# DoubangoTelecom/compv

Hardware: AMD Instinct MI355X
Metric: Mpixels/s Sobel->Canny->HoughSHT on 4K uint8 (higher is better)
Workload: dtype u8; 1 GPU; batched 3840x2160 uint8 frames, Sobel3x3 -> Canny(59,119) -> HoughSHT(rho=1, theta=1deg, thr=100); 256 distinct frames resident per GPU as 8 batches of 32, a step processes one batch, steps rotate over the batches; frames_per_gpu=32, resident_batches=8, parallelism=frames sharded across 1 GPU(s), no data-path collective

## Files before the change

compv_amd/csrc/api.cpp:

```cpp
#include "../../include/compv_hip.h"
#include "kernels.hpp"
#include "kht.hpp"

#include <atomic>
#include <chrono>
#include <condition_variable>
#include <deque>
#include <functional>
#include <mutex>
#include <thread>

#include <hip/hip_runtime.h>
#if defined(__linux__)
#include <sched.h>
#endif

#include <algorithm>
#include <cmath>
#include <cstdio>
#include <cstdlib>
#include <cstring>
#include <string>
#include <memory>
#include <vector>
// ... 101 lines not shown
};

struct StepParams {
	const uint8_t* d_in = nullptr; float tLow = 0.f, tHigh = 0.f; int threshold = 0, maxLines = 0;
	int ksize = 3, thresholdType = COMPVHIP_CANNY_THRESHOLD_COMPARE_TO_GRADIENT, pixfmt = COMPVHIP_FMT_Y;
	uint8_t* d_gray = nullptr; int32_t* d_otsu = nullptr; float* d_cart = nullptr;
	uint8_t* d_edges = nullptr; compvhip_line* d_lines = nullptr; size_t lineCap = 0; int32_t* d_counts = nullptr;
};

struct compvhip_plan : TimingState {
	compvhip_ctx* ctx = nullptr;
	size_t W = 0, H = 0, S = 0, frames = 0;
	float thetaDeg = 1.f;
	int tilesX = 0, tilesY = 0, wb = 0;
	size_t bitsFrameStride = 0;
	uint32_t* ebits = nullptr; uint32_t* ubits = nullptr;
	int* counters = nullptr;
	size_t nCounts = 0;
	int* flags = nullptr; int* hFlags = nullptr;
	int* frameTotals = nullptr; unsigned int* lineTotal = nullptr;
	unsigned int* hTotals = nullptr;
	unsigned int recentTotals[8] = {}; int recentN = 0;
	int specRounds = kSpecRounds; unsigned char recentRounds[8] = {}; int recentRoundsN = 0;
	int* hRoundsDev = nullptr; int* stepHostSlot = nullptr;
	int* hRounds = nullptr;
	int roundsUsed = 0;
	int maxRounds = kMaxRounds;
	bool countersFresh = false;
	int2* thrDev = nullptr; unsigned int* sums = nullptr;
	uint8_t* dirty = nullptr;
	uint8_t* patchOut = nullptr; uint8_t* copyBack = nullptr;
	uint8_t* grayTmp = nullptr;
	uint8_t* tmpOut = nullptr;
	bool bitsValid = false;
	bool shtReady = false;
	size_t R = 0, T = 0; float thetaStep = 0.f; int accPitch = 0;
	uint8_t* blurTmp = nullptr;
	uint32_t* hist = nullptr; int32_t* otsu = nullptr;
	float* cosT = nullptr; float* invSinT = nullptr;
	int32_t* sinQ = nullptr; int32_t* cosQ = nullptr;
	uint32_t* edges = nullptr; size_t edgeCap = 0; int* edgeCounts = nullptr;
	uint16_t* acc = nullptr; size_t accFrameStride = 0;
	uint32_t* keysA = nullptr; uint32_t* keysB = nullptr; uint32_t* valsA = nullptr; uint32_t* valsB = nullptr; size_t lineCap = 0; int* lineCounts = nullptr;
	int2* reach = nullptr;
	int2* nmsRange = nullptr;
	uint8_t* nmsFlags = nullptr;
	int* blockCounts = nullptr; int lineBlocks = 0;
	void* sortTemp = nullptr; size_t sortTempBytes = 0;
	int32_t* segPerLine = nullptr; size_t segPerLineCap = 0;
	int32_t* compRows = nullptr; uint32_t* compBits = nullptr; int32_t* compParent = nullptr;
	uint8_t* morphTmp = nullptr;
	int* fastWork = nullptr; uint8_t* fastScores = nullptr;
	int strengthBits = 16, keyBits = 0;
	uint16_t* chunkHist = nullptr; uint32_t* strengthStart = nullptr; int sortChunks = 0; bool deviceSort = false;
	bool voteTiles = false;
	ShtTileArgs vt = {};
	std::vector<int32_t> vtKt, vtRowBase;
	int32_t* dKt = nullptr; int32_t* dRowBase = nullptr; uint8_t* partLo = nullptr; uint8_t* partHi = nullptr; uint8_t* colFlag = nullptr; int* tileCounts = nullptr;
	std::vector<KhtBatchState*> khtBatch;
	std::vector<std::unique_ptr<KhtPeaksWork>> khtWork;
	double khtStageMs[6] = {}; double khtWallMs = 0.0; int khtThreads = 0;
	struct AsyncStep { bool used = false; bool replay = false; uint64_t seq = 0; hipEvent_t done = nullptr; hipStream_t stream = nullptr; StepParams sp; size_t sortN = 0; int rounds = 0; } steps[kAsyncDepth];
	uint64_t stepSeq = 0;
};

struct compvhip_matcher : TimingState {
	compvhip_ctx* ctx = nullptr;
	int descDwords = 0, queryCap = 0, trainCap = 0, pairs = 0, knn = 0;
	uint32_t* partial = nullptr;
	compvhip_match* reverse = nullptr;
};

namespace {

int fail(compvhip_ctx* ctx, int code, const char* what, hipError_t e = hipSuccess)
{
	if (ctx) {
		ctx->err = what ? what : "";
		if (e != hipSuccess) { ctx->err += ": "; ctx->err += hipGetErrorString(e); }
	}
	return code;
}

#define HIPCHK(ctx, call) do { hipError_t e__ = (call); if (e__ != hipSuccess) return fail((ctx), COMPVHIP_E_HIP, #call, e__); } while (0)

template <typename T>
hipError_t dmalloc(compvhip_ctx* ctx, T** p, size_t count)
{
	*p = nullptr;
	if (!count) return hipSuccess;
	hipError_t e = hipMalloc(reinterpret_cast<void**>(p), count * sizeof(T));
	if (e == hipSuccess && ctx) ctx->live++;
	return e;
}
template <typename T>
void dfree(compvhip_ctx* ctx, T*& p)
{
	if (p) { (void)hipFree(p); if (ctx) ctx->live--; p = nullptr; }
}

size_t alignUp(size_t v, size_t a) { return (v + a - 1) / a * a; }

void khtScratchFree(compvhip_ctx* ctx, KhtScratch& k)
{
	dfree(ctx, k.counts); dfree(ctx, k.params); dfree(ctx, k.cells); dfree(ctx, k.cellCount);
	dfree(ctx, k.pts); dfree(ctx, k.spans); dfree(ctx, k.kernelsDev);
	dfree(ctx, k.strings); dfree(ctx, k.counts32); dfree(ctx, k.scratch); dfree(ctx, k.stack);
// ... 263 lines not shown
				for (int i = 0; i < tiles; ++i) {
					const int b = p->vtRowBase[static_cast<size_t>(i) * T + t];
					lo = std::min(lo, b); hi = std::max(hi, b + Rw);
				}
				reach[t] = make_int2(lo, hi);
			}
			dfree(ctx, p->reach);
			HIPCHK(ctx, dmalloc(ctx, &p->reach, reach.size()));
			HIPCHK(ctx, hipMemcpy(p->reach, reach.data(), reach.size() * sizeof(int2), hipMemcpyHostToDevice));
			dfree(ctx, p->nmsRange);
			HIPCHK(ctx, dmalloc(ctx, &p->nmsRange, range.size()));
			HIPCHK(ctx, hipMemcpy(p->nmsRange, range.data(), range.size() * sizeof(int2), hipMemcpyHostToDevice));
		}
		HIPCHK(ctx, dmalloc(ctx, &p->dKt, p->vtKt.size()));
		HIPCHK(ctx, dmalloc(ctx, &p->dRowBase, p->vtRowBase.size()));
		HIPCHK(ctx, hipMemcpy(p->dKt, p->vtKt.data(), p->vtKt.size() * sizeof(int32_t), hipMemcpyHostToDevice));
		HIPCHK(ctx, hipMemcpy(p->dRowBase, p->vtRowBase.data(), p->vtRowBase.size() * sizeof(int32_t), hipMemcpyHostToDevice));
		{
			const size_t cols = p->frames * p->vt.tiles * static_cast<size_t>(p->vt.Tpad);
			HIPCHK(ctx, dmalloc(ctx, &p->partLo, cols * p->vt.rwPitch));
			HIPCHK(ctx, dmalloc(ctx, &p->partHi, cols * p->vt.rwPitch));
			HIPCHK(ctx, dmalloc(ctx, &p->colFlag, cols));
		}
		p->vt.kt = p->dKt; p->vt.rowBase = p->dRowBase; p->vt.partLo = p->partLo; p->vt.partHi = p->partHi; p->vt.colFlag = p->colFlag; p->vt.reach = p->reach; p->vt.tileCounts = p->tileCounts;
		p->edgeCap = static_cast<size_t>(p->vt.tiles) * p->vt.tileCap;
	}
	HIPCHK(ctx, dmalloc(ctx, &p->edges, p->edgeCap * p->frames));
	HIPCHK(ctx, dmalloc(ctx, &p->acc, p->accFrameStride * p->frames));
	HIPCHK(ctx, hipMemset(p->acc, 0, sizeof(uint16_t) * p->accFrameStride * p->frames));
	p->strengthBits = 1;
	while ((static_cast<size_t>(1) << p->strengthBits) <= 2 * (p->W > p->H ? p->W : p->H)) p->strengthBits++;
	if (p->strengthBits > 16) p->strengthBits = 16;
	int frameBits = 0;
	while ((static_cast<size_t>(1) << frameBits) < p->frames) frameBits++;
	p->keyBits = frameBits + p->strengthBits;
	if (R * T >= (static_cast<size_t>(1) << 32)) return fail(ctx, COMPVHIP_E_INVALID_PARAMETER, "theta step too small: the accumulator has 2^32 cells or more");
	if (p->keyBits > 32) return fail(ctx, COMPVHIP_E_INVALID_PARAMETER, "too many frames for a 32-bit line key");
	dfree(ctx, p->nmsFlags);
	{
		const size_t frows = sht_nms_rows(static_cast<int>(R)), fgroups = static_cast<size_t>(sht_nms_groups(static_cast<int>(T)));
		HIPCHK(ctx, dmalloc(ctx, &p->nmsFlags, frows * fgroups * p->frames));
		HIPCHK(ctx, hipMemset(p->nmsFlags, 0, frows * fgroups * p->frames));
		if (sht_lines_blocks(static_cast<int>(R)) != p->lineBlocks) return fail(ctx, COMPVHIP_E_INVALID_STATE, "row-block counters were sized for another accumulator");
	}
	p->shtReady = true;
	return COMPVHIP_OK;
}

int ensureLineCap(compvhip_plan* p, size_t cap)
{
	compvhip_ctx* ctx = p->ctx;
	cap = std::min(cap, p->R * p->T);
	if (cap <= p->lineCap) return COMPVHIP_OK;
	dfree(ctx, p->keysA); dfree(ctx, p->keysB); dfree(ctx, p->valsA); dfree(ctx, p->valsB); dfree(ctx, p->sortTemp); dfree(ctx, p->chunkHist); dfree(ctx, p->strengthStart);
	p->lineCap = 0; p->deviceSort = false;
	HIPCHK(ctx, dmalloc(ctx, &p->keysA, cap * p->frames));
	HIPCHK(ctx, dmalloc(ctx, &p->keysB, cap * p->frames));
	HIPCHK(ctx, dmalloc(ctx, &p->valsA, cap * p->frames));
	HIPCHK(ctx, dmalloc(ctx, &p->valsB, cap * p->frames));
	size_t tb = 0;
	hipError_t e = sht_sort_pairs(nullptr, tb, p->keysA, p->keysB, p->valsA, p->valsB, cap * p->frames, p->keyBits, nullptr);
	if (e != hipSuccess) return fail(ctx, COMPVHIP_E_HIP, "radix sort size query", e);
	p->sortTempBytes = tb;
	uint8_t* tmp = nullptr;
	HIPCHK(ctx, dmalloc(ctx, &tmp, std::max<size_t>(tb, 16)));
	p->sortTemp = tmp;
	p->sortChunks = static_cast<int>((cap + kShtSortChunk - 1) / kShtSortChunk);
	if (p->strengthBits <= kShtSortMaxStrengthBits && p->sortChunks <= kShtSortMaxChunks) {
		HIPCHK(ctx, dmalloc(ctx, &p->chunkHist, p->frames * static_cast<size_t>(p->sortChunks) << kShtSortMaxStrengthBits));
		HIPCHK(ctx, dmalloc(ctx, &p->strengthStart, p->frames << kShtSortMaxStrengthBits));
		p->deviceSort = true;
	}
	p->lineCap = cap;
	p->recentN = 0;
	return COMPVHIP_OK;
}

ShtArgs shtArgs(compvhip_plan* p, int threshold)
{
	ShtArgs a;
	a.ebits = p->ebits; a.edges = p->edges; a.edgeCounts = p->edgeCounts; a.acc = p->acc;
	a.sinQ = p->sinQ; a.cosQ = p->cosQ; a.lineKeys = p->keysA; a.lineVals = p->valsA; a.lineCounts = p->lineCounts;
	a.frameTotals = p->frameTotals; a.lineTotal = p->lineTotal; a.sortN = 0; a.outCounts = nullptr; a.stepFlags = nullptr; a.hostStep = nullptr;
	a.nmsRange = p->nmsRange; a.blockCounts = p->blockCounts; a.lineBlocks = p->lineBlocks; a.nmsFlags = p->nmsFlags; a.nmsRows = static_cast<int>(sht_nms_rows(static_cast<int>(p->R))); a.nmsGroups = sht_nms_groups(static_cast<int>(p->T));
	a.bitsFrameStride = p->bitsFrameStride; a.edgeCap = p->edgeCap; a.accFrameStride = p->accFrameStride; a.lineCap = p->lineCap;
	a.W = static_cast<int>(p->W); a.H = static_cast<int>(p->H); a.wb = p->wb;
	a.R = static_cast<int>(p->R); a.T = static_cast<int>(p->T); a.accPitch = p->accPitch; a.barrier = static_cast<int>(p->W + p->H);
	a.threshold = threshold;
	a.nmsLastCol = static_cast<int>((p->T - 1) & ~static_cast<size_t>(3));
	a.frames = static_cast<int>(p->frames);
	a.strengthBits = p->strengthBits;
	return a;
}

int ensurePreproc(compvhip_plan* p)
{
	compvhip_ctx* ctx = p->ctx;
	if (!p->hist) HIPCHK(ctx, dmalloc(ctx, &p->hist, static_cast<size_t>(256) * kOtsuMaxChunks * p->frames));
	if (!p->otsu) HIPCHK(ctx, dmalloc(ctx, &p->otsu, p->frames));
	return COMPVHIP_OK;
}

int enqueueCanny(compvhip_plan* p, const uint8_t* d_in, uint8_t* d_out, int tLow, int tHigh, int ksize, int thrMode, float fLow, float fHigh, hipStream_t st)
{
	compvhip_ctx* ctx = p->ctx;
	CannyArgs a;
	a.zero = nullptr; a.nZero = 0;
	a.in = d_in; a.out = d_out; a.ebits = p->ebits; a.ubits = p->ubits; a.thrDev = (thrMode != COMPVHIP_CANNY_THRESHOLD_COMPARE_TO_GRADIENT) ? p->thrDev : nullptr;
	a.inFrameStride = p->S * p->H; a.outFrameStride = p->S * p->H; a.bitsFrameStride = p->bitsFrameStride;
	a.W = static_cast<int>(p->W); a.H = static_cast<int>(p->H); a.S = static_cast<int>(p->S); a.So = static_cast<int>(p->S);
	a.wb = p->wb; a.tilesX = p->tilesX; a.tilesY = p->tilesY; a.tLow = tLow; a.tHigh = tHigh; a.ksize = ksize;
	cannyCoverage(p->W, &a.simdEnd, &a.cStart);
	const bool gap = !((a.simdEnd >= a.W - 1) || (a.cStart <= a.simdEnd));
	if (thrMode == COMPVHIP_CANNY_THRESHOLD_OTSU) {
		int rc = ensurePreproc(p);
		if (rc) return rc;
		Stamp s(p, st, "otsu_kernels");
		HIPCHK(ctx, launch_otsu(d_in, a.W, a.H, a.S, a.inFrameStride, static_cast<int>(p->frames), fLow, fHigh, p->hist, p->otsu, p->thrDev, st));
	}
	if (thrMode == COMPVHIP_CANNY_THRESHOLD_PERCENT_OF_MEAN) {
		Stamp s(p, st, "canny_mean_thresholds");
		HIPCHK(ctx, launch_mean_thresholds(d_in, a.W, a.H, a.S, a.inFrameStride, static_cast<int>(p->frames), fLow, fHigh, p->sums, p->thrDev, st));
	}
// ... 320 lines not shown
		if (hipMemset(p->ebits, 0, sizeof(uint32_t) * p->bitsFrameStride * frames) != hipSuccess) { rc = COMPVHIP_E_HIP; break; }
		if (hipMemset(p->ubits, 0, sizeof(uint32_t) * p->bitsFrameStride * frames) != hipSuccess) { rc = COMPVHIP_E_HIP; break; }
		if (hipDeviceSynchronize() != hipSuccess) { rc = COMPVHIP_E_HIP; break; }
		{
			p->voteTiles = true;
			size_t R = 0, T = 0; float step = 0.f;
			if (p->voteTiles && shtDims(W, H, thetaDeg, &R, &T, &step) == COMPVHIP_OK && T >= 5) {
				std::vector<int32_t> sq, cq;
				shtTables(thetaDeg, T, sq, cq);
				if (!planVoteTiles(W, H, frames, sq, cq, p->vt, p->vtKt, p->vtRowBase)) p->voteTiles = false;
			}
			else p->voteTiles = false;
			p->lineBlocks = p->voteTiles ? sht_lines_blocks(static_cast<int>(R)) : 0;
			p->nCounts = (2 + static_cast<size_t>(p->voteTiles ? p->vt.tiles : 0) + static_cast<size_t>(p->lineBlocks)) * frames + (frames + 1) * kFrameSlot;
		}
		if (dmalloc(ctx, &p->counters, p->nCounts + kMaxRounds) != hipSuccess) { rc = COMPVHIP_E_OUT_OF_MEMORY; break; }
		p->edgeCounts = p->counters; p->lineCounts = p->counters + frames; p->tileCounts = p->counters + 2 * frames; p->blockCounts = p->counters + (2 + static_cast<size_t>(p->voteTiles ? p->vt.tiles : 0)) * frames; p->flags = p->counters + p->nCounts;
		p->frameTotals = p->blockCounts + static_cast<size_t>(p->lineBlocks) * frames; p->lineTotal = reinterpret_cast<unsigned int*>(p->frameTotals + frames * kFrameSlot);
		if (const char* e = getenv("COMPVHIP_RESOLVE_WRAP")) { const int v = atoi(e); if (v >= 8 && v <= kMaxRounds && (v & 3) == 0) p->maxRounds = v; }
		if (hipMemset(p->counters, 0, sizeof(int) * (p->nCounts + kMaxRounds)) != hipSuccess) { rc = COMPVHIP_E_HIP; break; }
		if (dmalloc(ctx, &p->thrDev, frames) != hipSuccess) { rc = COMPVHIP_E_OUT_OF_MEMORY; break; }
		if (dmalloc(ctx, &p->dirty, canny_resolve_dirty_bytes(static_cast<int>(H), p->wb, static_cast<int>(frames))) != hipSuccess) { rc = COMPVHIP_E_OUT_OF_MEMORY; break; }
		if (dmalloc(ctx, &p->sums, frames * kFrameSlot) != hipSuccess) { rc = COMPVHIP_E_OUT_OF_MEMORY; break; }
		if (hipHostMalloc(reinterpret_cast<void**>(&p->hFlags), sizeof(int) * 2 * (kAsyncDepth + 1)) != hipSuccess) { rc = COMPVHIP_E_OUT_OF_MEMORY; break; }
		p->hTotals = reinterpret_cast<unsigned int*>(p->hFlags + kAsyncDepth + 1);
		if (hipHostMalloc(reinterpret_cast<void**>(&p->hRounds), sizeof(int) * (kFrameSlot + 4) * kAsyncDepth, hipHostMallocMapped) != hipSuccess) { rc = COMPVHIP_E_OUT_OF_MEMORY; break; }
		if (hipHostGetDevicePointer(reinterpret_cast<void**>(&p->hRoundsDev), p->hRounds, 0) != hipSuccess) { rc = COMPVHIP_E_HIP; break; }
	} while (0);
	if (rc) { compvhip_plan_destroy(p); return fail(ctx, rc, "plan allocation"); }
	*out = p;
	return COMPVHIP_OK;
}

void compvhip_plan_destroy(compvhip_plan* p)
{
	if (!p) return;
	compvhip_ctx* ctx = p->ctx;
	(void)hipSetDevice(ctx->device);
	timelineClear(p);
	for (hipEvent_t e : p->eventPool) (void)hipEventDestroy(e);
	for (auto& stp : p->steps) if (stp.done) (void)hipEventDestroy(stp.done);
	dfree(ctx, p->dirty);
	dfree(ctx, p->ebits); dfree(ctx, p->ubits); dfree(ctx, p->counters); dfree(ctx, p->thrDev); dfree(ctx, p->sums); dfree(ctx, p->tmpOut);
	if (p->hFlags) (void)hipHostFree(p->hFlags);
	if (p->hRounds) (void)hipHostFree(p->hRounds);
	dfree(ctx, p->hist); dfree(ctx, p->otsu); dfree(ctx, p->blurTmp); dfree(ctx, p->grayTmp);
	dfree(ctx, p->morphTmp);
	dfree(ctx, p->fastWork); dfree(ctx, p->fastScores);
	for (KhtBatchState* b : p->khtBatch) khtBatchFree(ctx, b);
	p->khtBatch.clear();
	dfree(ctx, p->cosT); dfree(ctx, p->invSinT);
	dfree(ctx, p->dKt); dfree(ctx, p->dRowBase); dfree(ctx, p->partLo); dfree(ctx, p->partHi); dfree(ctx, p->colFlag);
	dfree(ctx, p->sinQ); dfree(ctx, p->cosQ); dfree(ctx, p->edges); dfree(ctx, p->acc);
	dfree(ctx, p->keysA); dfree(ctx, p->keysB); dfree(ctx, p->valsA); dfree(ctx, p->valsB); dfree(ctx, p->nmsFlags); dfree(ctx, p->chunkHist); dfree(ctx, p->strengthStart);
	dfree(ctx, p->nmsRange); dfree(ctx, p->reach); dfree(ctx, p->sortTemp); dfree(ctx, p->segPerLine);
	dfree(ctx, p->compRows); dfree(ctx, p->compBits); dfree(ctx, p->compParent);
	delete p;
}

int compvhip_plan_set_timing(compvhip_plan* p, int enabled)
{
	if (!p) return COMPVHIP_E_INVALID_PARAMETER;
	p->timing = (enabled >= 2 && enabled <= 4) ? enabled : (enabled != 0 ? 1 : 0);
	return COMPVHIP_OK;
}

int compvhip_plan_get_timing(compvhip_plan* p, const char** names, float* ms, int cap)
{
	if (!p) return COMPVHIP_E_INVALID_PARAMETER;
	(void)hipSetDevice(p->ctx->device);
	if (!p->timeline.empty()) {
		for (auto& t : p->timeline) (void)hipEventSynchronize(t.b);
		timelineCollect(p);
	}
	const int n = std::min<int>(cap, static_cast<int>(p->timingMs.size()));
	for (int i = 0; i < n; ++i) { if (names) names[i] = p->timingNames[i].c_str(); if (ms) ms[i] = p->timingMs[i]; }
	return n;
}

static int planCannyImpl(compvhip_plan* p, const uint8_t* d_in, float tLow, float tHigh, int ksize, int type, uint8_t* d_edges, hipStream_t st,
                         bool waitConverged, bool clearTimeline = true)
{
	compvhip_ctx* ctx = p->ctx;
	if (!d_in || !d_edges) return fail(ctx, COMPVHIP_E_INVALID_PARAMETER, "null frame pointer");
	int lo, hi;
	int rc = validateCannyParams(ctx, tLow, tHigh, ksize, type, &lo, &hi);
	if (rc) return rc;
	HIPCHK(ctx, hipSetDevice(ctx->device));
	if (p->timing && clearTimeline) timelineClear(p);
	uint8_t* out = d_edges;
	const size_t bytes = p->S * p->H * p->frames;
	const bool alias = (d_in < d_edges + bytes) && (d_edges < d_in + bytes);
	if (alias) {
		if (!p->tmpOut) HIPCHK(ctx, dmalloc(ctx, &p->tmpOut, bytes));
		out = p->tmpOut;
	}
	p->patchOut = out;
	p->copyBack = alias ? d_edges : nullptr;
	if (p->W < static_cast<size_t>(ksize) || p->H < static_cast<size_t>(ksize)) return fail(ctx, COMPVHIP_E_INVALID_PARAMETER, "image smaller than the kernel");
	rc = enqueueCanny(p, d_in, out, lo, hi, ksize, type, tLow, tHigh, st);
	if (rc) return rc;
	rc = enqueueResolve(p, p->patchOut, waitConverged ? kSpecRounds : p->specRounds, st);
	if (rc) return rc;
	if (waitConverged) {
		for (;;) {
			bool done = false;
			rc = resolveConverged(p, st, &done);
// ... 94 lines not shown
	hipStream_t st = static_cast<hipStream_t>(stream);
	if (p->timing) timelineClear(p);
	EdgeDeteArgs a;
	a.in = d_in; a.out = d_out; a.gmax = p->sums;
	a.inFrameStride = p->S * p->H; a.outFrameStride = p->S * p->H;
	a.W = static_cast<int>(p->W); a.H = static_cast<int>(p->H); a.S = static_cast<int>(p->S); a.So = static_cast<int>(p->S);
	a.tilesX = p->tilesX; a.tilesY = p->tilesY;
	Stamp s(p, st, "edge_dete_kernels");
	HIPCHK(ctx, launch_edge_dete(a, op, static_cast<int>(p->frames), st));
	return COMPVHIP_OK;
}

constexpr size_t kSortAll = ~static_cast<size_t>(0), kSortExact = kSortAll - 1;

static int planShtImpl(compvhip_plan* p, const uint8_t* d_edges, int threshold, int maxLines, compvhip_line* d_lines, size_t lineCap, int32_t* d_counts,
                       hipStream_t st, bool clearTimeline, bool pairsOnly = false, size_t sortN = kSortAll)
{
	compvhip_ctx* ctx = p->ctx;
	if (threshold <= 0) return fail(ctx, COMPVHIP_E_INVALID_PARAMETER, "threshold must be > 0");
	if (!d_edges && !p->bitsValid) return fail(ctx, COMPVHIP_E_INVALID_STATE, "no edge masks: run compvhip_plan_canny first or pass d_edges");
	HIPCHK(ctx, hipSetDevice(ctx->device));
	int rc = ensureSht(p);
	if (rc) return rc;
	rc = ensureLineCap(p, std::max(lineCap, kMinLineCap));
	if (rc) return rc;
	if (p->timing && clearTimeline) timelineClear(p);
	const int frames = static_cast<int>(p->frames);
	if (d_edges) {
		Stamp s(p, st, "bytes_to_bits_kernel");
		HIPCHK(ctx, launch_bytes_to_bits(d_edges, static_cast<int>(p->W), static_cast<int>(p->H), static_cast<int>(p->S), p->S * p->H, p->ebits, p->wb,
		                                 p->bitsFrameStride, frames, st));
		p->bitsValid = false;
	}
	ShtArgs a = shtArgs(p, threshold);
	a.outCounts = d_counts;
	a.hostStep = p->stepHostSlot; a.stepFlags = p->flags;
	const size_t capAll = p->lineCap * p->frames;
	const bool deviceSort = p->deviceSort && !pairsOnly;
	if (sortN != kSortExact) sortN = std::min(sortN, capAll);
	a.sortN = (pairsOnly || deviceSort || sortN == kSortExact) ? 0 : sortN;
	if (!p->countersFresh) HIPCHK(ctx, hipMemsetAsync(p->counters, 0, sizeof(int) * p->nCounts, st));
	p->countersFresh = false;
	{ Stamp s(p, st, "sht_compact_kernel"); HIPCHK(ctx, launch_sht_compact_tiles(a, p->vt, frames, st)); }
	{ Stamp s(p, st, "sht_vote_kernel"); HIPCHK(ctx, launch_sht_vote_tiles(a, p->vt, frames, st)); }
	{ Stamp s(p, st, "sht_reduce_kernel"); HIPCHK(ctx, launch_sht_reduce_tiles(a, p->vt, frames, st)); }
	{ Stamp s(p, st, "sht_lines_kernel"); HIPCHK(ctx, launch_sht_lines(a, frames, st)); }
	if (pairsOnly) {
		return COMPVHIP_OK;
	}
	if (deviceSort) {
		if (d_lines && lineCap) {
			Stamp s(p, st, "sht_sort_lines");
			ShtSortArgs q;
			q.sortedKeys = p->keysB; q.sortedVals = p->valsB; q.chunkHist = p->chunkHist; q.strengthStart = p->strengthStart; q.chunks = p->sortChunks;
			HIPCHK(ctx, launch_sht_sort_lines(a, q, frames, p->thetaStep, maxLines, d_lines, lineCap, st));
		}
		return COMPVHIP_OK;
	}
	if (sortN == kSortExact) {
		HIPCHK(ctx, hipMemcpyAsync(p->hTotals, p->lineTotal, sizeof(unsigned int), hipMemcpyDeviceToHost, st));
		HIPCHK(ctx, hipStreamSynchronize(st));
		sortN = std::min(static_cast<size_t>(p->hTotals[0]), capAll);
	}
	if (sortN) {
		Stamp s(p, st, "sht_sort_lines");
		size_t tb = p->sortTempBytes;
		hipError_t e = sht_sort_pairs(p->sortTemp, tb, p->keysA, p->keysB, p->valsA, p->valsB, sortN, p->keyBits, st);
		if (e != hipSuccess) return fail(ctx, COMPVHIP_E_HIP, "radix sort", e);
	}
	if (d_lines && lineCap) {
		Stamp s(p, st, "sht_decode_kernel");
		HIPCHK(ctx, launch_sht_decode(p->keysB, p->valsB, p->lineCounts, p->lineCap, frames, static_cast<int>(p->T), static_cast<int>(p->W + p->H), p->thetaStep, maxLines,
		                              p->strengthBits, d_lines, lineCap, st));
	}
	return COMPVHIP_OK;
}

int compvhip_plan_houghsht(compvhip_plan* p, const uint8_t* d_edges, int threshold, int maxLines, compvhip_line* d_lines, size_t lineCap,
                           int32_t* d_counts, void* stream)
{
	if (!p) return COMPVHIP_E_INVALID_PARAMETER;
	return planShtImpl(p, d_edges, threshold, maxLines, d_lines, lineCap, d_counts, static_cast<hipStream_t>(stream), true);
}

static int checkStep(compvhip_plan* p, const StepParams& sp)
{
	compvhip_ctx* ctx = p->ctx;
	if (!sp.d_in || !sp.d_edges) return fail(ctx, COMPVHIP_E_INVALID_PARAMETER, "null frame pointer");
	if (sp.pixfmt != COMPVHIP_FMT_Y) {
		if (!pixfmtBytes(sp.pixfmt)) return fail(ctx, COMPVHIP_E_NOT_IMPLEMENTED, "pixel format without a grayscale conversion");
		if ((sp.pixfmt == COMPVHIP_FMT_YUYV422 || sp.pixfmt == COMPVHIP_FMT_UYVY422) && (p->W & 1))
			return fail(ctx, COMPVHIP_E_INVALID_PARAMETER, "packed 4:2:2 needs an even width");
	}
	if (sp.d_cart && (!sp.d_lines || !sp.d_counts)) return fail(ctx, COMPVHIP_E_INVALID_PARAMETER, "toCartesian needs the line and count buffers");
	return COMPVHIP_OK;
}

static int enqueueStep(compvhip_plan* p, const StepParams& sp, hipStream_t st, bool clearTimeline)
{
	compvhip_ctx* ctx = p->ctx;
	HIPCHK(ctx, hipSetDevice(ctx->device));
	const uint8_t* luma = sp.d_in;
	if (sp.pixfmt != COMPVHIP_FMT_Y) {
		uint8_t* gray = sp.d_gray;
		if (!gray) {
			if (!p->grayTmp) HIPCHK(ctx, dmalloc(ctx, &p->grayTmp, p->S * p->H * p->frames));
			gray = p->grayTmp;
// ... 1871 lines not shown
```

compv_amd/csrc/kernels.hpp:

```cpp
#pragma once
#include <hip/hip_runtime.h>
#include <stddef.h>
#include <stdint.h>

#include "../../include/compv_hip.h"

namespace compvhip {

#ifndef COMPVHIP_BAND_H
#define COMPVHIP_BAND_H 64
#endif
constexpr int kBandH = COMPVHIP_BAND_H;
#ifndef COMPVHIP_BAND_WORDS
#define COMPVHIP_BAND_WORDS 64
#endif
constexpr int kBandWords = COMPVHIP_BAND_WORDS;
constexpr int kResolveThreads = 512;
constexpr int kFrameSlot = 32;
constexpr int kResolveRows = kBandH * kBandWords / kResolveThreads;

struct CannyArgs {
	const uint8_t* in;
	uint8_t* out;
	uint32_t* ebits;
// ... 83 lines not shown
	int* blockCounts;
	int lineBlocks;
	const int2* nmsRange;
	int nmsGroups;
	int* lineCounts;
	const int* stepFlags;
	int* hostStep;
	int32_t* outCounts;
	int* frameTotals;
	unsigned int* lineTotal;
	size_t sortN;
	size_t bitsFrameStride, edgeCap, accFrameStride, lineCap;
	int W, H, wb;
	int R, T, accPitch, barrier;
	int threshold, nmsLastCol;
	int frames;
	int strengthBits;
};
struct ShtTileArgs {
	const int32_t* kt;
	const int32_t* rowBase;
	uint8_t* partLo;
	uint8_t* partHi;
	uint8_t* colFlag;
	const int2* reach;
	int* tileCounts;
	int nx, ny, TW, TH, tiles;
	int Rw, rwPitch;
	int Tpad, groups;
	size_t tileCap;
};
constexpr int kShtMaxWindow = 1264;
hipError_t launch_sht_compact_tiles(const ShtArgs& a, const ShtTileArgs& v, int frames, hipStream_t stream);
hipError_t launch_sht_vote_tiles(const ShtArgs& a, const ShtTileArgs& v, int frames, hipStream_t stream);
hipError_t launch_sht_reduce_tiles(const ShtArgs& a, const ShtTileArgs& v, int frames, hipStream_t stream);
hipError_t launch_bytes_to_bits(const uint8_t* edges, int W, int H, int S, size_t frameStride, uint32_t* ebits, int wb, size_t bitsFrameStride,
                                int frames, hipStream_t stream);
hipError_t launch_sht_lines(const ShtArgs& a, int frames, hipStream_t stream);
hipError_t launch_sht_decode(const uint32_t* keys, const uint32_t* vals, const int* counts, size_t lineCap, int frames, int T, int barrier, float thetaStep,
                             int maxLines, int strengthBits, void* lines , size_t outCap, hipStream_t stream);
int sht_nms_groups(int T);
size_t sht_nms_rows(int R);
int sht_lines_blocks(int R);
hipError_t launch_sht_cartesian(const void* lines , const int* counts, size_t lineCap, int maxLines, int frames, int T, const float* cosT,
                                const float* invSinT, float thetaStep, float widthF, float r, float* out , hipStream_t stream);
hipError_t launch_sht_acc_transpose(const uint16_t* accT, int R, int T, int accPitch, int32_t* out, size_t outStride, hipStream_t stream);
constexpr int kShtSortChunk = 4096;
constexpr int kShtSortMaxStrengthBits = 13;
constexpr int kShtSortMaxChunks = 32;
struct ShtSortArgs {
	uint32_t* sortedKeys;
	uint32_t* sortedVals;
	uint16_t* chunkHist;
	uint32_t* strengthStart;
	int chunks;
};
hipError_t launch_sht_sort_lines(const ShtArgs& a, const ShtSortArgs& q, int frames, float thetaStep, int maxLines, void* lines , size_t outCap,
                                 hipStream_t stream);
hipError_t sht_sort_pairs(void* temp, size_t& tempBytes, const uint32_t* keysIn, uint32_t* keysOut, const uint32_t* valsIn, uint32_t* valsOut, size_t n,
                          int keyBits, hipStream_t stream);

struct ShtSegArgs {
	const uint32_t* ebits;
	const uint8_t* edges;
	size_t bitsFrameStride, edgeFrameStride;
	int wb, S;
	const int32_t* sinQ;
	const int32_t* cosQ;
	const compvhip_line* lines;
	const int32_t* lineCounts;
	size_t lineCap;
	int nLines;
	int W, H, R, T, barrier;
	int minLength, maxGap;
	int32_t* perLine;
	compvhip_segment* segs;
	size_t segCap;
	int32_t* segCounts;
	int frame0;
};
hipError_t launch_sht_segments(const ShtSegArgs& a, int frames, int phase, hipStream_t stream);

struct ShtFitArgs {
	const uint32_t* ebits;
	const uint8_t* edges;
	size_t bitsFrameStride, edgeFrameStride;
	int wb, S;
	const int32_t* sinQ;
	const int32_t* cosQ;
	const compvhip_line* lines;
	const int32_t* lineCounts;
	size_t lineCap;
	int nLines;
	int W, H, R, T, barrier;
	int halfWidth;
	const compvhip_segment* segs;
	const int32_t* segCounts;
	size_t segCap;
	compvhip_line_fit* fits;
	size_t fitCap;
	int32_t* fitCounts;
	compvhip_line* refined;
	int frame0;
};
hipError_t launch_sht_fit(const ShtFitArgs& a, int frames, hipStream_t stream);

struct CompArgs {
// ... 103 lines not shown
```

compv_amd/csrc/sht_sort_kernels.hip:

```cpp
#include "kernels.hpp"

#include <type_traits>

namespace compvhip {

namespace {

constexpr int kChunk = kShtSortChunk;
constexpr int kSortThreads = 1024;
constexpr int kBins = 1 << kShtSortMaxStrengthBits;
static_assert(kChunk == 4096 && kBins == 8192, "key layout: 13 bits of inverted strength above 12 bits of chunk position");

struct LineOut { float rho; float theta; int32_t strength; int32_t row; int32_t col; };

template <int THREADS>
__device__ __forceinline__ size_t frame_base(const int* __restrict__ counts, int frame, size_t lineCap, unsigned long long* s_part)
{
	unsigned long long before = 0;
	for (int g = threadIdx.x; g < frame; g += THREADS) {
		const size_t cg = (size_t)max(counts[g], 0);
		before += cg < lineCap ? cg : lineCap;
	}
#pragma unroll
	for (int d = 32; d > 0; d >>= 1) before += __shfl_xor(before, d);
	if ((threadIdx.x & 63) == 0) s_part[threadIdx.x >> 6] = before;
	__syncthreads();
	unsigned long long sum = 0;
#pragma unroll
	for (int w = 0; w < THREADS / 64; ++w) sum += s_part[w];
	return (size_t)sum;
}

}

__global__ __launch_bounds__(kSortThreads) void sht_chunk_sort_kernel(ShtArgs a, ShtSortArgs q)
{
	__shared__ uint32_t s_key[kChunk];
	__shared__ uint32_t s_hist[kBins];
	__shared__ uint32_t s_cnt[kSortThreads], s_wsum[kSortThreads / 64];
	__shared__ unsigned long long s_part[kSortThreads / 64];
	const int frame = blockIdx.y, chunk = blockIdx.x, t = threadIdx.x;
	const size_t nf = min((size_t)max(a.lineCounts[frame], 0), a.lineCap);
	const size_t c0 = (size_t)chunk * kChunk;
	if (c0 >= nf) return;
	const int m = (int)min((size_t)kChunk, nf - c0);
	const size_t base = frame_base<kSortThreads>(a.lineCounts, frame, a.lineCap, s_part) + c0;
	const uint32_t mask = (1u << a.strengthBits) - 1u;
	const uint32_t* __restrict__ kin = a.lineKeys + base;
	const uint32_t* __restrict__ vin = a.lineVals + base;
	uint32_t e[4];
	{
		uint32_t kraw[4];
#pragma unroll
		for (int u = 0; u < 4; ++u) kraw[u] = kin[min(u * kSortThreads + t, m - 1)];
		asm volatile("" : "+v"(kraw[0]), "+v"(kraw[1]), "+v"(kraw[2]), "+v"(kraw[3]));
#pragma unroll
		for (int u = 0; u < 4; ++u) {
			const int i = u * kSortThreads + t;
			e[u] = i < m ? (((mask - (kraw[u] & mask)) << 12) | (uint32_t)i) : 0xffffffffu;
		}
	}
#pragma unroll
	for (int u = 0; u < kBins / kSortThreads; ++u) s_hist[t + u * kSortThreads] = 0u;
	const int lane = t & 63, wave = t >> 6;
// ... 29 lines not shown
		uint32_t before = 0;
#pragma unroll
		for (int w = 0; w < kSortThreads / 64; ++w) before += (w < wave) ? s_wsum[w] : 0u;
		s_cnt[t] = before + incl - c;
		__syncthreads();
#pragma unroll
		for (int u = 0; u < 4; ++u) s_key[s_cnt[slot[u]] + rank[u]] = e[u];
		__syncthreads();
#pragma unroll
		for (int u = 0; u < 4; ++u) e[u] = s_key[u * kSortThreads + t];
	};
	radix_pass(std::integral_constant<int, 4>{}, 12);
	radix_pass(std::integral_constant<int, 3>{}, 16);
	radix_pass(std::integral_constant<int, 3>{}, 19);
	radix_pass(std::integral_constant<int, 3>{}, 22);
	uint32_t* __restrict__ kout = q.sortedKeys + base;
	uint32_t* __restrict__ vout = q.sortedVals + base;
	{
		uint32_t kk[4]; int lo[4], hi[4];
#pragma unroll
		for (int u = 0; u < 4; ++u) { const int i = min(t + u * kSortThreads, m - 1); kk[u] = s_key[i]; lo[u] = 0; hi[u] = i; }
#pragma unroll
		for (int s = 0; s < 12; ++s) {
#pragma unroll
			for (int u = 0; u < 4; ++u) {
				const int mid = (lo[u] + hi[u]) >> 1;
				const bool ge = s_key[mid] >= (kk[u] & ~4095u);
				hi[u] = ge ? mid : hi[u];
				lo[u] = ge ? lo[u] : mid + 1;
			}
		}
		uint32_t cell[4];
#pragma unroll
		for (int u = 0; u < 4; ++u) cell[u] = vin[kk[u] & 4095u];
		asm volatile("" : "+v"(cell[0]), "+v"(cell[1]), "+v"(cell[2]), "+v"(cell[3]));
#pragma unroll
		for (int u = 0; u < 4; ++u) {
			const int i = t + u * kSortThreads;
			if (i < m) {
				kout[i] = (kk[u] & ~4095u) | (uint32_t)(i - lo[u]);
				vout[i] = cell[u];
				atomicAdd(&s_hist[kk[u] >> 12], 1u);
			}
		}
	}
	__syncthreads();
	uint4* __restrict__ hout = reinterpret_cast<uint4*>(q.chunkHist + ((size_t)frame * q.chunks + chunk) * kBins);
	{
		const uint32_t* h = s_hist + 8 * t;
		hout[t] = make_uint4(h[0] | (h[1] << 16), h[2] | (h[3] << 16), h[4] | (h[5] << 16), h[6] | (h[7] << 16));
	}
}

__global__ __launch_bounds__(kSortThreads) void sht_strength_scan_kernel(ShtArgs a, ShtSortArgs q)
{
	__shared__ uint32_t s_wave[kSortThreads / 64];
	const int frame = blockIdx.x, t = threadIdx.x;
	const size_t nf = min((size_t)max(a.lineCounts[frame], 0), a.lineCap);
	if (nf == 0) return;
	const int nch = (int)((nf + kChunk - 1) / kChunk);
	uint32_t tot[8] = { 0, 0, 0, 0, 0, 0, 0, 0 };
	const uint4* __restrict__ h = reinterpret_cast<const uint4*>(q.chunkHist + (size_t)frame * q.chunks * kBins) + t;
	auto add8 = [](uint32_t (&d)[8], const uint4& v) {
		d[0] += v.x & 0xffffu; d[1] += v.x >> 16; d[2] += v.y & 0xffffu; d[3] += v.y >> 16;
		d[4] += v.z & 0xffffu; d[5] += v.z >> 16; d[6] += v.w & 0xffffu; d[7] += v.w >> 16;
	};
	const uint4 zero4 = make_uint4(0u, 0u, 0u, 0u);
	for (int c0 = 0; c0 < nch; c0 += 4) {
		uint4 v[4];
#pragma unroll
		for (int u = 0; u < 4; ++u) v[u] = h[(size_t)min(c0 + u, nch - 1) * (kBins / 8)];
#pragma unroll
		for (int u = 0; u < 4; ++u) add8(tot, (c0 + u < nch) ? v[u] : zero4);
	}
	uint32_t sum = 0;
#pragma unroll
	for (int u = 0; u < 8; ++u) { const uint32_t c = tot[u]; tot[u] = sum; sum += c; }
	uint32_t incl = sum;
	const int lane = t & 63, wave = t >> 6;
#pragma unroll
	for (int o = 1; o < 64; o <<= 1) {
		const uint32_t n = __shfl_up(incl, o);
		if (lane >= o) incl += n;
	}
	if (lane == 63) s_wave[wave] = incl;
	__syncthreads();
	uint32_t before = 0;
#pragma unroll
	for (int w = 0; w < kSortThreads / 64; ++w) before += (w < wave) ? s_wave[w] : 0u;
	const uint32_t excl = before + incl - sum;
	uint4* __restrict__ out = reinterpret_cast<uint4*>(q.strengthStart + (size_t)frame * kBins) + 2 * t;
	out[0] = make_uint4(excl + tot[0], excl + tot[1], excl + tot[2], excl + tot[3]);
	out[1] = make_uint4(excl + tot[4], excl + tot[5], excl + tot[6], excl + tot[7]);
}

__global__ __launch_bounds__(256) void sht_place_lines_kernel(ShtArgs a, ShtSortArgs q, float thetaStep, int maxLines, LineOut* __restrict__ lines, size_t outCap)
{
	__shared__ unsigned long long s_part[4];
	const int frame = blockIdx.y;
	const size_t nf = min((size_t)max(a.lineCounts[frame], 0), a.lineCap);
	const size_t i0 = (size_t)blockIdx.x * 256;
	if (i0 >= nf) return;
	const size_t base = frame_base<256>(a.lineCounts, frame, a.lineCap, s_part);
	const size_t i = i0 + threadIdx.x;
	if (i >= nf) return;
	size_t limit = nf;
	if (maxLines > 0 && limit > (size_t)maxLines) limit = (size_t)maxLines;
	if (limit > outCap) limit = outCap;
	const uint32_t kv = q.sortedKeys[base + i];
	const uint32_t inv = kv >> 12, rank = kv & 4095u;
	const int c = (int)(i >> 12);
	size_t pos = (size_t)q.strengthStart[(size_t)frame * kBins + inv] + rank;
	const uint16_t* __restrict__ h = q.chunkHist + (size_t)frame * q.chunks * kBins + inv;
	for (int c0 = 0; c0 < c; c0 += 4) {
		uint32_t v[4];
#pragma unroll
		for (int u = 0; u < 4; ++u) v[u] = h[(size_t)min(c0 + u, c) * kBins];
#pragma unroll
		for (int u = 0; u < 4; ++u) pos += (c0 + u < c) ? v[u] : 0u;
	}
	if (pos >= limit) return;
	const uint32_t cell = q.sortedVals[base + i];
	const int row = (int)(cell / (uint32_t)a.T), col = (int)(cell - (uint32_t)row * (uint32_t)a.T);
	LineOut o;
	o.rho = (float)(a.barrier - row);
	o.theta = __fmul_rn((float)col, thetaStep);
	o.strength = (int32_t)(((1u << a.strengthBits) - 1u) - inv);
	o.row = row; o.col = col;
	lines[(size_t)frame * outCap + pos] = o;
}

hipError_t launch_sht_sort_lines(const ShtArgs& a, const ShtSortArgs& q, int frames, float thetaStep, int maxLines, void* lines, size_t outCap, hipStream_t stream)
{
	if (!lines || !outCap) return hipSuccess;
	hipLaunchKernelGGL(sht_chunk_sort_kernel, dim3((unsigned)q.chunks, (unsigned)frames), dim3(kSortThreads), 0, stream, a, q);
	hipLaunchKernelGGL(sht_strength_scan_kernel, dim3((unsigned)frames), dim3(kSortThreads), 0, stream, a, q);
	hipLaunchKernelGGL(sht_place_lines_kernel, dim3((unsigned)(q.chunks * (kChunk / 256)), (unsigned)frames), dim3(256), 0, stream, a, q, thetaStep, maxLines,
	                   reinterpret_cast<LineOut*>(lines), outCap);
	return hipGetLastError();
}

}
```

Before: 427,100 Mpixels/s.

## Fuse strength scan into line placement kernel, drop strengthStart buffer

Merges the per-frame strength prefix-scan kernel into the line placement kernel. Each chunk block recomputes the per-frame scan, adds the counts from earlier chunks, stages the offsets through a shared-memory table in four passes, and places its 4096 lines. This removes one kernel launch, the global strengthStart buffer round trip, and the per-line serial loop over earlier chunks' histograms. In exchange every chunk block rereads the whole frame histogram and repeats the scan, which is redundant work when there are many chunks.

```diff
diff --git a/compv_amd/csrc/api.cpp b/compv_amd/csrc/api.cpp
--- a/compv_amd/csrc/api.cpp
+++ b/compv_amd/csrc/api.cpp
@@ -177,7 +177,7 @@
 	uint8_t* morphTmp = nullptr;
 	int* fastWork = nullptr; uint8_t* fastScores = nullptr;
 	int strengthBits = 16, keyBits = 0;
-	uint16_t* chunkHist = nullptr; uint32_t* strengthStart = nullptr; int sortChunks = 0; bool deviceSort = false;
+	uint16_t* chunkHist = nullptr; int sortChunks = 0; bool deviceSort = false;
 	bool voteTiles = false;
 	ShtTileArgs vt = {};
 	std::vector<int32_t> vtKt, vtRowBase;
@@ -547,7 +547,7 @@
 	compvhip_ctx* ctx = p->ctx;
 	cap = std::min(cap, p->R * p->T);
 	if (cap <= p->lineCap) return COMPVHIP_OK;
-	dfree(ctx, p->keysA); dfree(ctx, p->keysB); dfree(ctx, p->valsA); dfree(ctx, p->valsB); dfree(ctx, p->sortTemp); dfree(ctx, p->chunkHist); dfree(ctx, p->strengthStart);
+	dfree(ctx, p->keysA); dfree(ctx, p->keysB); dfree(ctx, p->valsA); dfree(ctx, p->valsB); dfree(ctx, p->sortTemp); dfree(ctx, p->chunkHist);
 	p->lineCap = 0; p->deviceSort = false;
 	HIPCHK(ctx, dmalloc(ctx, &p->keysA, cap * p->frames));
 	HIPCHK(ctx, dmalloc(ctx, &p->keysB, cap * p->frames));
@@ -563,7 +563,6 @@
 	p->sortChunks = static_cast<int>((cap + kShtSortChunk - 1) / kShtSortChunk);
 	if (p->strengthBits <= kShtSortMaxStrengthBits && p->sortChunks <= kShtSortMaxChunks) {
 		HIPCHK(ctx, dmalloc(ctx, &p->chunkHist, p->frames * static_cast<size_t>(p->sortChunks) << kShtSortMaxStrengthBits));
-		HIPCHK(ctx, dmalloc(ctx, &p->strengthStart, p->frames << kShtSortMaxStrengthBits));
 		p->deviceSort = true;
 	}
 	p->lineCap = cap;
@@ -990,7 +989,7 @@
 	dfree(ctx, p->cosT); dfree(ctx, p->invSinT);
 	dfree(ctx, p->dKt); dfree(ctx, p->dRowBase); dfree(ctx, p->partLo); dfree(ctx, p->partHi); dfree(ctx, p->colFlag);
 	dfree(ctx, p->sinQ); dfree(ctx, p->cosQ); dfree(ctx, p->edges); dfree(ctx, p->acc);
-	dfree(ctx, p->keysA); dfree(ctx, p->keysB); dfree(ctx, p->valsA); dfree(ctx, p->valsB); dfree(ctx, p->nmsFlags); dfree(ctx, p->chunkHist); dfree(ctx, p->strengthStart);
+	dfree(ctx, p->keysA); dfree(ctx, p->keysB); dfree(ctx, p->valsA); dfree(ctx, p->valsB); dfree(ctx, p->nmsFlags); dfree(ctx, p->chunkHist);
 	dfree(ctx, p->nmsRange); dfree(ctx, p->reach); dfree(ctx, p->sortTemp); dfree(ctx, p->segPerLine);
 	dfree(ctx, p->compRows); dfree(ctx, p->compBits); dfree(ctx, p->compParent);
 	delete p;
@@ -1191,7 +1190,7 @@
 		if (d_lines && lineCap) {
 			Stamp s(p, st, "sht_sort_lines");
 			ShtSortArgs q;
-			q.sortedKeys = p->keysB; q.sortedVals = p->valsB; q.chunkHist = p->chunkHist; q.strengthStart = p->strengthStart; q.chunks = p->sortChunks;
+			q.sortedKeys = p->keysB; q.sortedVals = p->valsB; q.chunkHist = p->chunkHist; q.chunks = p->sortChunks;
 			HIPCHK(ctx, launch_sht_sort_lines(a, q, frames, p->thetaStep, maxLines, d_lines, lineCap, st));
 		}
 		return COMPVHIP_OK;
diff --git a/compv_amd/csrc/kernels.hpp b/compv_amd/csrc/kernels.hpp
--- a/compv_amd/csrc/kernels.hpp
+++ b/compv_amd/csrc/kernels.hpp
@@ -159,7 +159,6 @@
 	uint32_t* sortedKeys;
 	uint32_t* sortedVals;
 	uint16_t* chunkHist;
-	uint32_t* strengthStart;
 	int chunks;
 };
 hipError_t launch_sht_sort_lines(const ShtArgs& a, const ShtSortArgs& q, int frames, float thetaStep, int maxLines, void* lines , size_t outCap,
diff --git a/compv_amd/csrc/sht_sort_kernels.hip b/compv_amd/csrc/sht_sort_kernels.hip
--- a/compv_amd/csrc/sht_sort_kernels.hip
+++ b/compv_amd/csrc/sht_sort_kernels.hip
@@ -10,6 +10,9 @@
 constexpr int kSortThreads = 1024;
 constexpr int kBins = 1 << kShtSortMaxStrengthBits;
 static_assert(kChunk == 4096 && kBins == 8192, "key layout: 13 bits of inverted strength above 12 bits of chunk position");
+constexpr int kPlaceTab = 2048;
+constexpr int kPlaceTabOwnersLog2 = 8;
+static_assert(kBins == 8 * kSortThreads && kPlaceTab == 8 << kPlaceTabOwnersLog2 && kChunk == 4 * kSortThreads, "a thread owns 8 strengths and 4 lines");
 
 struct LineOut { float rho; float theta; int32_t strength; int32_t row; int32_t col; };
 
@@ -145,30 +148,47 @@
 	}
 }
 
-__global__ __launch_bounds__(kSortThreads) void sht_strength_scan_kernel(ShtArgs a, ShtSortArgs q)
-{
+__global__ __launch_bounds__(kSortThreads) __attribute__((amdgpu_waves_per_eu(8, 8))) void sht_place_lines_kernel(ShtArgs a, ShtSortArgs q, float thetaStep, int maxLines, LineOut* __restrict__ lines, size_t outCap)
+{
+	__shared__ __attribute__((aligned(16))) uint32_t s_tab[kPlaceTab];
 	__shared__ uint32_t s_wave[kSortThreads / 64];
-	const int frame = blockIdx.x, t = threadIdx.x;
+	__shared__ unsigned long long s_part[kSortThreads / 64];
+	const int frame = blockIdx.y, chunk = blockIdx.x, t = threadIdx.x;
 	const size_t nf = min((size_t)max(a.lineCounts[frame], 0), a.lineCap);
-	if (nf == 0) return;
+	const size_t c0 = (size_t)chunk * kChunk;
+	if (c0 >= nf) return;
+	const int m = (int)min((size_t)kChunk, nf - c0);
 	const int nch = (int)((nf + kChunk - 1) / kChunk);
-	uint32_t tot[8] = { 0, 0, 0, 0, 0, 0, 0, 0 };
+	size_t limit = nf;
+	if (maxLines > 0 && limit > (size_t)maxLines) limit = (size_t)maxLines;
+	if (limit > outCap) limit = outCap;
+	const size_t base = frame_base<kSortThreads>(a.lineCounts, frame, a.lineCap, s_part) + c0;
+	uint32_t kv[4], cell[4];
+#pragma unroll
+	for (int u = 0; u < 4; ++u) {
+		const size_t i = base + (size_t)min(t + u * kSortThreads, m - 1);
+		kv[u] = q.sortedKeys[i]; cell[u] = q.sortedVals[i];
+	}
+	uint32_t tot[8] = { 0, 0, 0, 0, 0, 0, 0, 0 }, bef[8] = { 0, 0, 0, 0, 0, 0, 0, 0 };
 	const uint4* __restrict__ h = reinterpret_cast<const uint4*>(q.chunkHist + (size_t)frame * q.chunks * kBins) + t;
 	auto add8 = [](uint32_t (&d)[8], const uint4& v) {
 		d[0] += v.x & 0xffffu; d[1] += v.x >> 16; d[2] += v.y & 0xffffu; d[3] += v.y >> 16;
 		d[4] += v.z & 0xffffu; d[5] += v.z >> 16; d[6] += v.w & 0xffffu; d[7] += v.w >> 16;
 	};
 	const uint4 zero4 = make_uint4(0u, 0u, 0u, 0u);
-	for (int c0 = 0; c0 < nch; c0 += 4) {
+	for (int g0 = 0; g0 < nch; g0 += 4) {
 		uint4 v[4];
 #pragma unroll
-		for (int u = 0; u < 4; ++u) v[u] = h[(size_t)min(c0 + u, nch - 1) * (kBins / 8)];
-#pragma unroll
-		for (int u = 0; u < 4; ++u) add8(tot, (c0 + u < nch) ? v[u] : zero4);
+		for (int u = 0; u < 4; ++u) v[u] = h[(size_t)min(g0 + u, nch - 1) * (kBins / 8)];
+#pragma unroll
+		for (int u = 0; u < 4; ++u) {
+			add8(tot, (g0 + u < nch) ? v[u] : zero4);
+			add8(bef, (g0 + u < chunk) ? v[u] : zero4);
+		}
 	}
 	uint32_t sum = 0;
 #pragma unroll
-	for (int u = 0; u < 8; ++u) { const uint32_t c = tot[u]; tot[u] = sum; sum += c; }
+	for (int u = 0; u < 8; ++u) { const uint32_t c = tot[u]; tot[u] = sum + bef[u]; sum += c; }
 	uint32_t incl = sum;
 	const int lane = t & 63, wave = t >> 6;
 #pragma unroll
@@ -182,53 +202,41 @@
 #pragma unroll
 	for (int w = 0; w < kSortThreads / 64; ++w) before += (w < wave) ? s_wave[w] : 0u;
 	const uint32_t excl = before + incl - sum;
-	uint4* __restrict__ out = reinterpret_cast<uint4*>(q.strengthStart + (size_t)frame * kBins) + 2 * t;
-	out[0] = make_uint4(excl + tot[0], excl + tot[1], excl + tot[2], excl + tot[3]);
-	out[1] = make_uint4(excl + tot[4], excl + tot[5], excl + tot[6], excl + tot[7]);
-}
-
-__global__ __launch_bounds__(256) void sht_place_lines_kernel(ShtArgs a, ShtSortArgs q, float thetaStep, int maxLines, LineOut* __restrict__ lines, size_t outCap)
-{
-	__shared__ unsigned long long s_part[4];
-	const int frame = blockIdx.y;
-	const size_t nf = min((size_t)max(a.lineCounts[frame], 0), a.lineCap);
-	const size_t i0 = (size_t)blockIdx.x * 256;
-	if (i0 >= nf) return;
-	const size_t base = frame_base<256>(a.lineCounts, frame, a.lineCap, s_part);
-	const size_t i = i0 + threadIdx.x;
-	if (i >= nf) return;
-	size_t limit = nf;
-	if (maxLines > 0 && limit > (size_t)maxLines) limit = (size_t)maxLines;
-	if (limit > outCap) limit = outCap;
-	const uint32_t kv = q.sortedKeys[base + i];
-	const uint32_t inv = kv >> 12, rank = kv & 4095u;
-	const int c = (int)(i >> 12);
-	size_t pos = (size_t)q.strengthStart[(size_t)frame * kBins + inv] + rank;
-	const uint16_t* __restrict__ h = q.chunkHist + (size_t)frame * q.chunks * kBins + inv;
-	for (int c0 = 0; c0 < c; c0 += 4) {
-		uint32_t v[4];
-#pragma unroll
-		for (int u = 0; u < 4; ++u) v[u] = h[(size_t)min(c0 + u, c) * kBins];
-#pragma unroll
-		for (int u = 0; u < 4; ++u) pos += (c0 + u < c) ? v[u] : 0u;
-	}
-	if (pos >= limit) return;
-	const uint32_t cell = q.sortedVals[base + i];
-	const int row = (int)(cell / (uint32_t)a.T), col = (int)(cell - (uint32_t)row * (uint32_t)a.T);
-	LineOut o;
-	o.rho = (float)(a.barrier - row);
-	o.theta = __fmul_rn((float)col, thetaStep);
-	o.strength = (int32_t)(((1u << a.strengthBits) - 1u) - inv);
-	o.row = row; o.col = col;
-	lines[(size_t)frame * outCap + pos] = o;
+	uint32_t pos[4] = { 0, 0, 0, 0 };
+#pragma unroll 1
+	for (int p = 0; p < kBins / kPlaceTab; ++p) {
+		if (p) __syncthreads();
+		if ((t >> kPlaceTabOwnersLog2) == p) {
+			uint4* o = reinterpret_cast<uint4*>(s_tab + 8 * (t & ((1 << kPlaceTabOwnersLog2) - 1)));
+			o[0] = make_uint4(excl + tot[0], excl + tot[1], excl + tot[2], excl + tot[3]);
+			o[1] = make_uint4(excl + tot[4], excl + tot[5], excl + tot[6], excl + tot[7]);
+		}
+		__syncthreads();
+#pragma unroll
+		for (int u = 0; u < 4; ++u) {
+			const uint32_t inv = kv[u] >> 12;
+			if ((int)(inv / kPlaceTab) == p) pos[u] = s_tab[inv % kPlaceTab] + (kv[u] & 4095u);
+		}
+	}
+#pragma unroll
+	for (int u = 0; u < 4; ++u) {
+		if (t + u * kSortThreads >= m || pos[u] >= limit) continue;
+		const uint32_t inv = kv[u] >> 12;
+		const int row = (int)(cell[u] / (uint32_t)a.T), col = (int)(cell[u] - (uint32_t)row * (uint32_t)a.T);
+		LineOut o;
+		o.rho = (float)(a.barrier - row);
+		o.theta = __fmul_rn((float)col, thetaStep);
+		o.strength = (int32_t)(((1u << a.strengthBits) - 1u) - inv);
+		o.row = row; o.col = col;
+		lines[(size_t)frame * outCap + pos[u]] = o;
+	}
 }
 
 hipError_t launch_sht_sort_lines(const ShtArgs& a, const ShtSortArgs& q, int frames, float thetaStep, int maxLines, void* lines, size_t outCap, hipStream_t stream)
 {
 	if (!lines || !outCap) return hipSuccess;
 	hipLaunchKernelGGL(sht_chunk_sort_kernel, dim3((unsigned)q.chunks, (unsigned)frames), dim3(kSortThreads), 0, stream, a, q);
-	hipLaunchKernelGGL(sht_strength_scan_kernel, dim3((unsigned)frames), dim3(kSortThreads), 0, stream, a, q);
-	hipLaunchKernelGGL(sht_place_lines_kernel, dim3((unsigned)(q.chunks * (kChunk / 256)), (unsigned)frames), dim3(256), 0, stream, a, q, thetaStep, maxLines,
+	hipLaunchKernelGGL(sht_place_lines_kernel, dim3((unsigned)q.chunks, (unsigned)frames), dim3(kSortThreads), 0, stream, a, q, thetaStep, maxLines,
 	                   reinterpret_cast<LineOut*>(lines), outCap);
 	return hipGetLastError();
 }
```

Result: slower. 421,500 Mpixels/s (-1.3%).
